# lamortenera/bamsignals

Measured on AMD Instinct MI355X. Metric: Mbases profiled/sec (bamProfile binsize=1), higher is better.
Workload: dtype int32

## Files before the change

### bamsignals_amd/csrc/bsig_types.h

```cpp
#ifndef BSIG_TYPES_H
#define BSIG_TYPES_H
#include <stdint.h>

#define BSIG_MAX_CLASSES 5
#define BSIG_SPAN_CLASSES 4
#define BSIG_CLASS_PACKED 4
#define BSIG_PACK_POS_BITS 15
#define BSIG_PACK_CODES 512
#define BSIG_REF_UNIT_SHIFT 16

struct BsigClassCols {
    const int32_t *pos;
    const int32_t *end;
    const uint32_t *fm;
    const int32_t *tlen;
    const uint32_t *idx;
    int64_t n;
    int32_t maxspan;
    int32_t kshift;
};

struct BsigReadsDev {
    BsigClassCols cls[BSIG_MAX_CLASSES];
    const uint32_t *fmtab;
    int32_t n_codes;
};

struct BsigWorkItem {
    int32_t loc;
    int32_t len;
// ... 18 lines not shown
    uint32_t requiredF;
    uint32_t filteredF;
    int32_t has_tlen_filter;
    int32_t tf0, tf1;
    int32_t use_tlen;
    int32_t shift;
    int32_t midpoint;
    int32_t tspan;
    int32_t ss;
    int32_t binsize;
    uint32_t div_magic;
    int32_t div_shift;
    uint32_t div_m15;
    int32_t div_s15;
    int32_t rel24;
    int32_t ext;
    int32_t tile_cells;
    int32_t accumulate;
    int32_t resolved;
    int32_t cov_reps;
    const uint8_t *ptab;
    int32_t *overflow;
};

#endif
```

### bamsignals_amd/csrc/kernels.h

```cpp
#ifndef BSIG_KERNELS_H
#define BSIG_KERNELS_H
#include <hip/hip_runtime.h>
#include <stdint.h>

#include "../../include/bamsignals_abi.h"
#include "bsig_types.h"

namespace bsig {

struct ScatterPtrs {
    int32_t *pos[BSIG_MAX_CLASSES];
    int32_t *end[BSIG_MAX_CLASSES];
    uint32_t *fm[BSIG_MAX_CLASSES];
    int32_t *tlen[BSIG_MAX_CLASSES];
    uint32_t *gb[BSIG_MAX_CLASSES];
    int32_t kshift[BSIG_MAX_CLASSES];
};

hipError_t launch_pileup(int mode, int ss, int threads, const BsigReadsDev &R, const BsigKParams &P,
                         const BsigWorkItem *items, int64_t n_items, int tile_cells,
                         void *windows ,
                         bool resolve_first ,
                         int32_t *out, hipStream_t st);
hipError_t launch_make_ptab(const BsigReadsDev &R, const BsigKParams &P, uint8_t *out, hipStream_t st);
hipError_t launch_resolve(const BsigReadsDev &R, const BsigKParams &P, int mode, const BsigWorkItem *items,
                          int64_t n_items, void *windows, hipStream_t st);
hipError_t launch_count_heavy(const void *windows, int64_t n_items, int64_t heavy_reads,
                              unsigned long long *count, hipStream_t st);
hipError_t launch_cigar_end(int64_t n, const int32_t *pos, const uint16_t *flag, const int64_t *cigar_off,
                            const uint32_t *cigar, int32_t *end_out, hipStream_t st);
int64_t prep_chunks(int64_t n);
hipError_t launch_pair_sample(int64_t n, const int32_t *pos, const int32_t *end, const uint16_t *flag, const uint8_t *mapq,
                              uint32_t *hist, uint2 *pairs, uint32_t cap, uint32_t *n_pairs, hipStream_t st);
hipError_t launch_codemap_fill(const uint32_t *fmtab, int n_codes, uint16_t *codemap, hipStream_t st);
hipError_t launch_span_hist(int64_t n, int32_t n_ref, const int64_t *ref_off, const uint32_t *ref_units, const int32_t *pos,
                            const int32_t *end, const uint16_t *flag, const uint8_t *mapq, const uint16_t *codemap ,
                            uint32_t *chunk_counts,
                            int32_t *maxspan , hipStream_t st);
// ... 15 lines not shown
```

### bamsignals_amd/csrc/kernels.hip

```cpp
#include <hip/hip_runtime.h>
#include <type_traits>
#include <stdint.h>
#include <stdlib.h>

#include <algorithm>

#include "bsig_types.h"
#include "kernels.h"

#ifdef BSIG_STAMPS
__device__ unsigned long long *g_stamp_buf = nullptr;
__device__ int g_ablate = 0;
#define BSIG_STAMP(k)                                                                       \
    do {                                                                                    \
        if (g_stamp_buf && threadIdx.x == 0) {                                              \
            unsigned long long t_;                                                          \
            asm volatile("s_memrealtime %0\n\ts_waitcnt lgkmcnt(0)" : "=s"(t_)::"memory");    \
            g_stamp_buf[(size_t)blockIdx.x * 8 + (k)] = t_;                                 \
        }                                                                                   \
    } while (0)
#define BSIG_ABLATE(bit) (g_ablate & (bit))
#else
#define BSIG_STAMP(k) do { } while (0)
#define BSIG_ABLATE(bit) 0
// ... 96 lines not shown
            if (TL) {
                const int a = tl < 0 ? -tl : tl;
                if (P.has_tlen_filter) rj |= ((a < P.tf0) | (a > P.tf1)) ? 0xFFFFFFFFu : 0u;
                if (P.midpoint) h = (uint32_t)(a >> 1);
            }
            const uint32_t fwd = d + h + (nm & (sp + cd - 2u * h));
            const uint32_t lc = (REV ? (uint32_t)K - fwd : (uint32_t)K + fwd) | rj;
            const bool ok = (dj + k < nj) & (lc < (uint32_t)nc);
            const uint32_t cell = SS ? (uint32_t)sh + 2u * lc + ((REV ? ~nm : nm) & 1u) : (uint32_t)sh + lc;
            if (ok) atomicAdd(&cnt[cell >> 1], 1u << ((cell << 4) & 31u));
        };
        rd(w.x, b0, t.x, 0u);
        rd(w.y, b1, t.y, 1u);
        rd(w.z, b2, t.z, 2u);
        rd(w.w, b3, t.w, 3u);
    }
};

template <bool SS>
struct SmallOne {
    const BsigKParams &P;
    int32_t *mine;
    int loc, len, c0, nc;
    bool neg_range;
    __device__ __forceinline__ void operator()(int p, int e, bool neg, bool rej, int tl, bool valid) const
    {
        constexpr int S = SS ? 2 : 1;
        if (!valid || rej || tlen_rejected(P, tl)) return;
        const int a = tl < 0 ? -tl : tl;
        const int offset = P.midpoint ? (a >> 1) + P.shift : P.shift;
// ... 206 lines not shown
    }
}
__global__ __launch_bounds__(128) void k_make_ptab(const BsigReadsDev R, const BsigKParams P, uint8_t *__restrict__ out)
{
    const int v = threadIdx.x;
    uint32_t word = 0;
    if (4 * v < R.n_codes) {
        const uint4 f = reinterpret_cast<const uint4 *>(R.fmtab)[v];
        auto b = [&](uint32_t fm) { return (uint32_t)fm_rejected(P, fm) | ((fm >> 3) & 2u); };
        word = b(f.x) | b(f.y) << 8 | b(f.z) << 16 | b(f.w) << 24;
    }
    reinterpret_cast<uint32_t *>(out)[v] = word;
}
static_assert(BSIG_PACK_CODES == 4 * 128, "k_make_ptab: four codes per thread of one 128-thread workgroup");

struct PackedWin {
    int base;
    int n_chunks;
};

__device__ __forceinline__ bool class_window(const BsigClassCols &C, const BsigWorkItem &w,
                                             int64_t tlo, int64_t thi, int ext,
                                             uint32_t &j_lo, uint32_t &j_hi)
{
    int64_t wlo = tlo - ext - C.maxspan + 1;
    int64_t whi = thi + ext;
    const int64_t ref_bp = (int64_t)(w.units_strand & BSIG_ITEM_UNITS_MASK) << BSIG_REF_UNIT_SHIFT;
    if (wlo < 0) wlo = 0;
    if (whi > ref_bp) whi = ref_bp;
    if (wlo >= whi) return false;
// ... 110 lines not shown
        else one.quad(w, t, j - j_lo, nj, base, ptab);
        return;
    }
    const uint32_t b0 = ptab[w.x >> 23], b1 = ptab[w.y >> 23], b2 = ptab[w.z >> 23], b3 = ptab[w.w >> 23];
    const uint32_t dj = j - j_lo;
    auto dec = [&](uint32_t x, uint32_t b, int tl, bool valid) {
        const int pos = base + (int)((x - (uint32_t)base) & kPackPosMask);
        one(pos, pos + (int)((x >> BSIG_PACK_POS_BITS) & 0xFFu), (b & 2u) != 0u, (b & 1u) != 0u, tl, valid);
    };
    dec(w.x, b0, t.x, dj < nj);
    dec(w.y, b1, t.y, dj + 1u < nj);
    dec(w.z, b2, t.z, dj + 2u < nj);
    dec(w.w, b3, t.w, dj + 3u < nj);
}

template <int NT, int kPre = 2, typename Tab, typename F>
__device__ __forceinline__ void for_each_read(const BsigReadsDev &R, const BsigKParams &P,
                                              const uint2 (&win)[BSIG_MAX_CLASSES], int pbase,
                                              const Tab *__restrict__ ptab, int tid, F &&one)
{
    uint4 w0[kPre];
    int4 t0[kPre];
    const BsigClassCols &CP = R.cls[BSIG_CLASS_PACKED];
    const uint32_t jbp = (win[BSIG_CLASS_PACKED].x & ~3u) + 4u * tid;
#pragma unroll
    for (int k = 0; k < kPre; ++k) {
        const uint32_t j = jbp + 4u * NT * k;
        if (j < win[BSIG_CLASS_PACKED].y) {
            w0[k] = *reinterpret_cast<const uint4 *>(CP.fm + j);
            if (P.use_tlen) t0[k] = *reinterpret_cast<const int4 *>(CP.tlen + j);
        }
    }
    const bool small0 = win[0].y - win[0].x <= (uint32_t)NT, small1 = win[1].y - win[1].x <= (uint32_t)NT;
    int pa = 0, ta = 0, pb = 0, tb = 0;
    uint32_t fa = 0, fb = 0;
    const uint32_t jb0 = win[0].x + (uint32_t)tid, jb1 = win[1].x + (uint32_t)tid;
    if (small0 && jb0 < win[0].y) {
        pa = R.cls[0].pos[jb0];
        fa = R.cls[0].fm[jb0];
        if (P.use_tlen) ta = R.cls[0].tlen[jb0];
    }
    if (small1 && jb1 < win[1].y) {
        pb = R.cls[1].pos[jb1];
        fb = R.cls[1].fm[jb1];
        if (P.use_tlen) tb = R.cls[1].tlen[jb1];
    }
    {
        const uint32_t j_lo = win[BSIG_CLASS_PACKED].x, j_hi = win[BSIG_CLASS_PACKED].y, nj = j_hi - j_lo;
        const uint32_t jp0 = j_lo & ~3u;
        auto inner_pass = [&](uint32_t first) { return first >= j_lo && first + 4u * NT <= j_hi; };
#pragma unroll
        for (int k = 0; k < kPre; ++k) {
            const uint32_t j = jbp + 4u * NT * k;
            if (j < j_hi) four_packed(w0[k], t0[k], j, j_lo, nj, pbase, ptab, one, inner_pass(jp0 + 4u * NT * k));
        }
        for (uint32_t j = jbp + 4u * NT * kPre, jf = jp0 + 4u * NT * kPre; j < j_hi; j += 8u * NT, jf += 8u * NT) {
            const uint32_t j2 = j + 4u * NT;
            const uint4 wa = *reinterpret_cast<const uint4 *>(CP.fm + j);
            int4 xa, xb;
            uint4 wb = make_uint4(0, 0, 0, 0);
            if (P.use_tlen) xa = *reinterpret_cast<const int4 *>(CP.tlen + j);
            if (j2 < j_hi) {
// ... 192 lines not shown
    for (int c = 0; c < BSIG_MAX_CLASSES; ++c) { r.win[2 * c] = win[c].x; r.win[2 * c + 1] = win[c].y; }
    r.pbase = pk.base;
    r.pchunks = pk.n_chunks;
    out[t] = r;
}

__device__ __forceinline__ void add_vec(int32_t *__restrict__ gbase, int v, int4 x, int sh, int nv)
{
    const int e0 = 4 * v, lo = sh, hi = sh + nv;
    if (x.x && e0 + 0 >= lo && e0 + 0 < hi) atomicAdd(gbase + e0 + 0, x.x);
    if (x.y && e0 + 1 >= lo && e0 + 1 < hi) atomicAdd(gbase + e0 + 1, x.y);
    if (x.z && e0 + 2 >= lo && e0 + 2 < hi) atomicAdd(gbase + e0 + 2, x.z);
    if (x.w && e0 + 3 >= lo && e0 + 3 < hi) atomicAdd(gbase + e0 + 3, x.w);
}

template <int NT, bool SS, int PRE, int WAVES, bool RES>
__global__ __launch_bounds__(NT) __attribute__((amdgpu_waves_per_eu(WAVES, 8))) void k_profile(const BsigWorkItem *__restrict__ items, uint32_t n_tiles,
                                                int32_t *__restrict__ out,
                                                const uint2 *__restrict__ windows,
                                                const BsigReadsDev R, const BsigKParams P)
{
    extern __shared__ __attribute__((aligned(16))) int32_t lds[];
    constexpr int S = SS ? 2 : 1;
    const int tid = threadIdx.x;
    BSIG_STAMP(0);
    const uint32_t tile = tile_of_block(blockIdx.x, n_tiles);
    const BsigWorkItem w = items[tile];
    uint2 win[BSIG_MAX_CLASSES], clip;
    PackedWin pk;
    load_windows<RES>(R, P, BSIG_MODE_PROFILE, w, items, windows, win, tile, pk, clip);
    int4 *lds4 = reinterpret_cast<int4 *>(lds);
    const int img_vec = (P.tile_cells * S + 8 + 7) / 8;
    for (int v = tid; v < img_vec; v += NT) lds4[v] = make_int4(0, 0, 0, 0);
    uint8_t *ptab = reinterpret_cast<uint8_t *>(lds4 + img_vec);
    build_ptab<NT>(ptab, R, P, tid);
    const int nv = w.nc * S;
    const int sh = (int)(w.out_off & 3);
    const int nvec = (sh + nv + 3) >> 2;
    block_sync<NT>();
    BSIG_STAMP(1);

    const bool neg_range = (w.units_strand & BSIG_ITEM_NEG) != 0u;
    uint32_t *cnt = reinterpret_cast<uint32_t *>(lds);

    const ProfileOne<SS> one{P, cnt, w.loc, w.len, w.c0, w.nc, sh, neg_range};
    if (!BSIG_ABLATE(1)) {
        for_each_read<NT, PRE>(R, P, win, pk.base, ptab, tid, one);
        if (pk.n_chunks > 1) packed_later_chunks<NT>(R, P, BSIG_MODE_PROFILE, w, pk.n_chunks, clip, ptab, tid, one);
    }
    block_sync<NT>();
    BSIG_STAMP(2);

    int32_t *gbase = out + (w.out_off - sh);
    const uint2 *lds2 = reinterpret_cast<const uint2 *>(lds);
    auto widen = [](uint2 d) {
        return make_int4((int)(d.x & 0xFFFFu), (int)(d.x >> 16), (int)(d.y & 0xFFFFu), (int)(d.y >> 16));
    };
    if (P.accumulate) {
        for (int v = tid; v < nvec; v += NT) add_vec(gbase, v, widen(lds2[v]), sh, nv);
    } else if (!BSIG_ABLATE(2)) {
        for (int v = tid; v < nvec; v += NT) store_vec(gbase, v, widen(lds2[v]), sh, nv);
    }
    BSIG_STAMP(3);
#ifdef BSIG_STAMPS
    asm volatile("s_waitcnt vmcnt(0)" ::: "memory");
    BSIG_STAMP(4);
    if (g_stamp_buf && threadIdx.x == 0) {
        unsigned xcc;
        asm volatile("s_getreg_b32 %0, hwreg(HW_REG_XCC_ID)" : "=s"(xcc));
        unsigned hwid;
        asm volatile("s_getreg_b32 %0, hwreg(HW_REG_HW_ID)" : "=s"(hwid));
        g_stamp_buf[(size_t)blockIdx.x * 8 + 5] = ((unsigned long long)xcc << 32) | hwid;
    }
#endif
}

template <bool SS, int PRE, int WAVES, int T>
__global__ __launch_bounds__(kWave) __attribute__((amdgpu_waves_per_eu(WAVES, 8))) void k_profile_multi(
    const BsigWorkItem *__restrict__ items, uint32_t n_tiles, int32_t *__restrict__ out, const uint2 *__restrict__ windows,
    const BsigReadsDev R, const BsigKParams P)
{
    extern __shared__ __attribute__((aligned(16))) int32_t lds[];
    constexpr int S = SS ? 2 : 1;
    constexpr int kStage = 20;
    const int tid = threadIdx.x;
    const uint32_t n_groups = (n_tiles + T - 1) / T;
    const uint32_t first = tile_of_block(blockIdx.x, n_groups) * T;
    const uint32_t n_here = n_tiles - first < (uint32_t)T ? n_tiles - first : (uint32_t)T;
    int4 *lds4 = reinterpret_cast<int4 *>(lds);
    const int img_vec = (P.tile_cells * S + 8 + 7) / 8;
    uint8_t *ptab = reinterpret_cast<uint8_t *>(lds4 + img_vec);
    uint32_t *stage = reinterpret_cast<uint32_t *>(ptab + BSIG_PACK_CODES);
    if ((uint32_t)tid < n_here) {
        const uint4 *ip = reinterpret_cast<const uint4 *>(items + first + tid);
        const uint4 *rp = reinterpret_cast<const uint4 *>(reinterpret_cast<const BsigResolved *>(windows) + first + tid);
        const uint4 a = ip[0], b = ip[1], c = rp[0], d = rp[1], e = rp[2];
        uint4 *sp = reinterpret_cast<uint4 *>(stage + kStage * tid);
        sp[0] = a; sp[1] = b; sp[2] = c; sp[3] = d; sp[4] = e;
    }
    for (int v = tid; v < img_vec; v += kWave) lds4[v] = make_int4(0, 0, 0, 0);
    build_ptab<kWave>(ptab, R, P, tid);
    block_sync<kWave>();
    uint32_t *cnt = reinterpret_cast<uint32_t *>(lds);
    uint2 *lds2 = reinterpret_cast<uint2 *>(lds);
#pragma unroll 1
    for (uint32_t t = 0; t < n_here; ++t) {
        const uint32_t *sg = stage + kStage * t;
        auto sc = [&](int k) { return __builtin_amdgcn_readfirstlane((int)sg[k]); };
        BsigWorkItem w;
        w.loc = sc(0); w.len = sc(1); w.c0 = sc(2); w.nc = sc(3);
        w.out_off = (int64_t)(((uint64_t)(uint32_t)sc(5) << 32) | (uint32_t)sc(4));
        w.ref_unit0 = (uint32_t)sc(6); w.units_strand = (uint32_t)sc(7);
        uint2 win[BSIG_MAX_CLASSES];
#pragma unroll
        for (int c = 0; c < BSIG_MAX_CLASSES; ++c) win[c] = make_uint2((uint32_t)sc(8 + 2 * c), (uint32_t)sc(9 + 2 * c));
        const int pbase = sc(18), pchunks = sc(19);
        const int nv = w.nc * S;
        const int sh = (int)(w.out_off & 3);
        const int nvec = (sh + nv + 3) >> 2;
        const bool neg_range = (w.units_strand & BSIG_ITEM_NEG) != 0u;
        const ProfileOne<SS> one{P, cnt, w.loc, w.len, w.c0, w.nc, sh, neg_range};
        for_each_read<kWave, PRE>(R, P, win, pbase, ptab, tid, one);
        if (pchunks > 1) packed_later_chunks<kWave>(R, P, BSIG_MODE_PROFILE, w, pchunks, make_uint2(0u, 0xFFFFFFFFu), ptab, tid, one);
        block_sync<kWave>();
        int32_t *gbase = out + (w.out_off - sh);
        for (int v = tid; v < nvec; v += kWave) {
            const uint2 d = lds2[v];
            lds2[v] = make_uint2(0u, 0u);
            store_vec(gbase, v, make_int4((int)(d.x & 0xFFFFu), (int)(d.x >> 16), (int)(d.y & 0xFFFFu), (int)(d.y >> 16)), sh, nv);
        }
        block_sync<kWave>();
    }
}

constexpr int kSmallCells = 256;
__host__ __device__ inline int small_replicas(int stride)
{
    return stride <= 32 ? 4 : stride <= 64 ? 2 : 1;
}
__host__ __device__ inline int small_image_dwords(int stride_max)
{
    int most = stride_max * small_replicas(stride_max);
    if (stride_max > 31) most = most > 31 * small_replicas(31) ? most : 31 * small_replicas(31);
    if (stride_max > 63) most = most > 63 * small_replicas(63) ? most : 63 * small_replicas(63);
    return most;
}
template <int NT, bool SS, bool RES>
// ... 718 lines not shown
                streamed += ((j_hi + 3u) & ~3u) - (j_lo & ~3u);
                const uint32_t x = lower_bound_packed(C.fm, j_lo, j_hi, a, wlo);
                const uint32_t y = lower_bound_packed(C.fm, x, j_hi, a, whi);
                v += y - x;
            }
            if (v) atomicAdd(&acc[BSIG_CLASS_PACKED], v);
        }
    }
    atomicAdd(&acc[BSIG_MAX_CLASSES], streamed);
}

}

namespace bsig {

static int g_knobs[6] = {-1, -1, -1, -1, -1, -1};
static int knob(int k)
{
    static const char *const names[6] = {"BAMSIGNALS_PROFILE_PRE", "BAMSIGNALS_COUNT_TILES", "BAMSIGNALS_COUNT_PRE", "BAMSIGNALS_KNOB3",
                                         "BAMSIGNALS_KNOB4", "BAMSIGNALS_PROFILE_TILES"};
    static const int dflt[6] = {2, 0, 0, 0, 0, 0};
    if (g_knobs[k] < 0) {
        const char *e = getenv(names[k]);
        g_knobs[k] = e ? atoi(e) : dflt[k];
    }
    return g_knobs[k];
}

template <int NT>
static hipError_t launch_mode(int mode, int ss, const BsigReadsDev &R, const BsigKParams &P,
                              const BsigWorkItem *items, int64_t n_items, int tile_cells,
                              uint2 *windows, bool resolve_first, int32_t *out, hipStream_t st)
{
    if (n_items <= 0) return hipSuccess;
    const bool count_large = n_items >= 65536;
    const int count_tiles = knob(1) > 0 ? knob(1) : count_large ? 8 : 4, count_pre = knob(2) > 0 ? knob(2) : count_large ? 4 : 2;
// ... 2 lines not shown
        Q.resolved = 0;
        hipLaunchKernelGGL(k_resolve_tiles, dim3((unsigned)((n_items + 255) / 256)), dim3(256), 0, st,
                           R, Q, mode, items, (uint32_t)n_items, reinterpret_cast<BsigResolved *>(windows));
    }
    const dim3 grid((unsigned)n_items), block(NT);
    if (mode == BSIG_MODE_PROFILE && tile_cells * (ss ? 2 : 1) <= kSmallCells && P.binsize > 1) {
        const int stride = (tile_cells * (ss ? 2 : 1)) | 1;
        const size_t lds = (size_t)((small_image_dwords(stride) + 3) & ~3) * sizeof(int32_t) + BSIG_PACK_CODES;
#define BSIG_KS(SS_, RES_) hipLaunchKernelGGL((k_profile_small<NT, SS_, RES_>), grid, block, lds, st, items, (uint32_t)n_items, out, windows, R, P)
        if (ss) { if (P.resolved) BSIG_KS(true, true); else BSIG_KS(true, false); }
        else    { if (P.resolved) BSIG_KS(false, true); else BSIG_KS(false, false); }
#undef BSIG_KS
    } else if (mode == BSIG_MODE_PROFILE) {
        const size_t lds = (size_t)((tile_cells * (ss ? 2 : 1) + 8 + 7) / 8) * 16 + BSIG_PACK_CODES;
        const int pre = knob(0);
#define BSIG_KP(SS_, PRE_, W_)                                                                                                          \
    do {                                                                                                                                \
        if (P.resolved) hipLaunchKernelGGL((k_profile<NT, SS_, PRE_, W_, true>), grid, block, lds, st, items, (uint32_t)n_items, out, windows, R, P); \
        else hipLaunchKernelGGL((k_profile<NT, SS_, PRE_, W_, false>), grid, block, lds, st, items, (uint32_t)n_items, out, windows, R, P); \
    } while (0)
        const bool w8 = NT == kWave && P.resolved && (knob(3) == 8 || (knob(3) == 0 && lds <= 3072));
        const int pt = knob(5) == 0 ? (lds <= 2048 ? 4 : 1) : knob(5);
        if (NT == kWave && P.resolved && !P.accumulate && pt > 1) {
            const int T = pt >= 4 ? 4 : 2;
            const dim3 g2((unsigned)((n_items + T - 1) / T));
            const size_t lds_m = lds + (size_t)T * 20 * sizeof(uint32_t);
#define BSIG_KM(SS_, W_, T_) hipLaunchKernelGGL((k_profile_multi<SS_, 2, W_, T_>), g2, dim3(kWave), lds_m, st, items, (uint32_t)n_items, out, windows, R, P)
            if (ss) { if (w8) { if (T == 4) BSIG_KM(true, 8, 4); else BSIG_KM(true, 8, 2); } else { if (T == 4) BSIG_KM(true, 1, 4); else BSIG_KM(true, 1, 2); } }
            else    { if (w8) { if (T == 4) BSIG_KM(false, 8, 4); else BSIG_KM(false, 8, 2); } else { if (T == 4) BSIG_KM(false, 1, 4); else BSIG_KM(false, 1, 2); } }
#undef BSIG_KM
            return hipGetLastError();
        }
        if (ss) { if (pre <= 2) { if (w8) BSIG_KP(true, 2, 8); else BSIG_KP(true, 2, 1); } else if (pre == 3) BSIG_KP(true, 3, 1); else BSIG_KP(true, 4, 1); }
        else    { if (pre <= 2) { if (w8) BSIG_KP(false, 2, 8); else BSIG_KP(false, 2, 1); } else if (pre == 3) BSIG_KP(false, 3, 1); else BSIG_KP(false, 4, 1); }
#undef BSIG_KP
    } else if (mode == BSIG_MODE_COVERAGE && (P.binsize > 1 || ss)) {
        const int S = ss ? 2 : 1;
        BsigKParams Q = P;
        Q.cov_reps = cov_bins_reps(tile_cells * S);
        const size_t lds = (size_t)cov_bins_vec(tile_cells * S) * Q.cov_reps * 16 + (size_t)((S * NT / 64 + 3) / 4) * 16 + BSIG_PACK_CODES;
#define BSIG_KB(RES_, SS_) hipLaunchKernelGGL((k_coverage_bins<NT, 2, RES_, SS_>), grid, block, lds, st, items, (uint32_t)n_items, out, windows, R, Q)
        if (ss) { if (P.resolved) BSIG_KB(true, true); else BSIG_KB(false, true); }
        else    { if (P.resolved) BSIG_KB(true, false); else BSIG_KB(false, false); }
#undef BSIG_KB
    } else if (mode == BSIG_MODE_COVERAGE) {
        const size_t lds = (size_t)((tile_cells + 8 + 7) / 8) * 16 + (size_t)((NT / 64 + 3) / 4) * 16 + BSIG_PACK_CODES;
        if (P.resolved) hipLaunchKernelGGL((k_coverage<NT, 2, true>), grid, block, lds, st, items, (uint32_t)n_items, out, windows, R, P);
        else hipLaunchKernelGGL((k_coverage<NT, 2, false>), grid, block, lds, st, items, (uint32_t)n_items, out, windows, R, P);
    } else if (NT == kWave && (!windows || P.resolved) && count_tiles > 1) {
// ... 16 lines not shown
{
    switch (threads) {
    case 64:  return launch_mode<64>(mode, ss, R, P, items, n_items, tile_cells, (uint2 *)windows, resolve_first, out, st);
    case 128: return launch_mode<128>(mode, ss, R, P, items, n_items, tile_cells, (uint2 *)windows, resolve_first, out, st);
    case 256: return launch_mode<256>(mode, ss, R, P, items, n_items, tile_cells, (uint2 *)windows, resolve_first, out, st);
    default:  return hipErrorInvalidValue;
    }
}

hipError_t launch_make_ptab(const BsigReadsDev &R, const BsigKParams &P, uint8_t *out, hipStream_t st)
{
    hipLaunchKernelGGL(k_make_ptab, dim3(1), dim3(128), 0, st, R, P, out);
    return hipGetLastError();
}

hipError_t launch_resolve(const BsigReadsDev &R, const BsigKParams &P, int mode, const BsigWorkItem *items,
                          int64_t n_items, void *windows, hipStream_t st)
{
    if (n_items <= 0) return hipSuccess;
    hipLaunchKernelGGL(k_resolve, dim3((unsigned)((n_items * BSIG_MAX_CLASSES + 255) / 256)), dim3(256), 0, st,
                       R, P, mode, items, n_items, (uint2 *)windows);
    return hipGetLastError();
}

hipError_t launch_count_heavy(const void *windows, int64_t n_items, int64_t heavy_reads,
                              unsigned long long *count, hipStream_t st)
{
    if (n_items <= 0) return hipSuccess;
    hipLaunchKernelGGL(k_count_heavy, dim3((unsigned)((n_items + 255) / 256)), dim3(256), 0, st,
                       (const uint2 *)windows, n_items, heavy_reads, count);
// ... 94 lines not shown
}

}

namespace { __global__ void k_warm_pileup() {} }
hipError_t bsig::warm_pileup_module(hipStream_t st)
{
    hipLaunchKernelGGL(k_warm_pileup, dim3(1), dim3(64), 0, st);
    return hipGetLastError();
}

extern "C" int bsig_debug_set_resolve_min(long long n_tiles);
extern "C" int bsig_debug_set_knob(int which, int value)
{
    if (which == 4) return bsig_debug_set_resolve_min(value);
    if (which < 0 || which >= 6 || value < 0) return -1;
    bsig::g_knobs[which] = value;
    return 0;
}

extern "C" int bsig_debug_pileup_attrs(int which, int *vgprs, int *scratch_bytes)
{
    const void *f = nullptr;
    switch (which) {
    case 0: f = reinterpret_cast<const void *>(&k_profile<64, false, 2, 1, true>); break;
    case 1: f = reinterpret_cast<const void *>(&k_profile<64, false, 2, 8, true>); break;
    case 2: f = reinterpret_cast<const void *>(&k_profile<64, false, 2, 1, false>); break;
    case 3: f = reinterpret_cast<const void *>(&k_profile_multi<false, 2, 8, 4>); break;
    case 4: f = reinterpret_cast<const void *>(&k_coverage<64, 2, true>); break;
    case 5: f = reinterpret_cast<const void *>(&k_count_multi<4, 2>); break;
    case 6: f = reinterpret_cast<const void *>(&k_profile<64, true, 2, 1, true>); break;
    default: return 1;
    }
    hipFuncAttributes a;
    if (hipFuncGetAttributes(&a, f) != hipSuccess) return 2;
    if (vgprs) *vgprs = a.numRegs;
    if (scratch_bytes) *scratch_bytes = (int)a.localSizeBytes;
    return 0;
}
#ifdef BSIG_STAMPS
extern "C" int bsig_debug_set_stamp_buffer(void *buf)
{
    return (int)hipMemcpyToSymbol(HIP_SYMBOL(g_stamp_buf), &buf, sizeof(buf));
}
extern "C" int bsig_debug_set_ablate(int bits)
{
// ... 4 lines not shown
```

### bamsignals_amd/csrc/runtime.hip

```cpp
#include <hip/hip_runtime.h>

#include <fcntl.h>
#include <sys/mman.h>
#include <sys/stat.h>
#include <unistd.h>

#include <algorithm>
#include <chrono>
#include <cstdarg>
#include <cstdio>
#include <cstdlib>
#include <cstring>
#include <atomic>
#include <functional>
#include <memory>
#include <mutex>
#include <numeric>
#include <thread>
#include <string>
#include <vector>

#include "../../include/bamsignals_abi.h"
#include "bsig_types.h"
#include "host_util.h"
// ... 350 lines not shown
    HIP_TRY(hipHostMalloc(ptr, (size_t)std::max<int64_t>(bytes, 16), hipHostMallocDefault));
    return BSIG_OK;
}

void bsig_host_free(void *ptr)
{
    if (ptr) (void)hipHostFree(ptr);
}

}

uint64_t bsig::next_layout_gen()
{
    static std::atomic<uint64_t> g{0};
    return ++g;
}

int bsig::layout_from_device(bsig_ctx *ctx, bsig_reads *R, int64_t n, int32_t n_ref, const int32_t *ref_len,
                             const int64_t *ref_off, const int32_t *d_pos, const int32_t *d_end,
                             const uint16_t *d_flag, const uint8_t *d_mapq, const int32_t *d_tlen)
{
    hipStream_t st = ctx->stream;
    HIP_TRY(hipSetDevice(ctx->device));
    R->layout_gen = next_layout_gen();

    R->n_ref = n_ref;
    R->ref_unit0.resize(n_ref);
    R->ref_units.resize(n_ref);
    R->ref_len.assign(ref_len, ref_len + n_ref);
    uint64_t total_units = 0;
// ... 136 lines not shown
        R->info.class_bucket_shift[c] = k;
        R->info.n_classes += 1;
    }
    R->info.n_codes = R->dev.n_codes;

    if (diag) fprintf(stderr, "  [layout] column + index allocations %.1f ms\n", diag_ms());
    HIP_TRY(bsig::launch_scatter(n, n_ref, d_ref_off, d_unit0, d_units, d_pos, d_end, d_flag, d_mapq, d_tlen, d_codemap,
                                 d_base, S, st));
    for (int c = 0; c < BSIG_MAX_CLASSES; ++c)
        if (class_n[c])
            HIP_TRY(bsig::launch_build_idx((int64_t)class_n[c], S.gb[c], n_buckets[c],
                                           const_cast<uint32_t *>(R->dev.cls[c].idx), st));
    HIP_TRY(hipStreamSynchronize(st));
    if (diag) fprintf(stderr, "  [layout] scatter + indexes %.1f ms\n", diag_ms());
    R->info.hbm_bytes = R->pool.footprint();
    return BSIG_OK;
}

extern "C" {

static int upload_impl(bsig_ctx *ctx, const bsig_columns *cols, bsig_reads *R)
{
    const int64_t n = cols->n_reads;
    hipStream_t st = ctx->stream;
    HIP_TRY(hipSetDevice(ctx->device));
    for (int r = 0; r < cols->n_ref; ++r)
        if (cols->ref_len[r] < 0) return fail(BSIG_ERR_ARG, "negative length of reference %d", r);
    if (n == 0 || cols->n_ref == 0)
        return bsig::layout_from_device(ctx, R, n, cols->n_ref, cols->ref_len, cols->ref_off, nullptr, nullptr, nullptr,
                                        nullptr, nullptr);
    DevPool tmp;
// ... 108 lines not shown
        copy(S.tlen, cb, &p); D.tlen = (const int32_t *)p;
        copy(S.idx, (size_t)src->idx_entries[c] * sizeof(uint32_t), &p); D.idx = (const uint32_t *)p;
    }
    {
        void *p;
        copy(src->dev.fmtab, BSIG_PACK_CODES * sizeof(uint32_t), &p);
        R->dev.fmtab = (const uint32_t *)p;
    }
    if (e == hipSuccess) e = hipStreamSynchronize(st);
    if (e != hipSuccess) {
        delete R;
        return fail(e == hipErrorOutOfMemory ? BSIG_ERR_NOMEM : BSIG_ERR_DEVICE, "copying the reads to GPU %d failed: %s", ddev,
                    hipGetErrorString(e));
    }
    R->info.hbm_bytes = R->pool.footprint();
    *out = R;
    return BSIG_OK;
}

}

namespace {

struct DownloadStage {
    std::mutex mu;
    hipEvent_t ev[2] = {nullptr, nullptr};
    static constexpr size_t kHalf = 32u << 20;
    int ensure()
    {
        for (int k = 0; k < 2; ++k)
// ... 484 lines not shown
        hipError_t e = hipMemsetAsync(d_bad, 0, sizeof(int), ctx->stream);
        for (int c = 0; c < BSIG_MAX_CLASSES && e == hipSuccess; ++c) {
            const BsigClassCols &C = R->dev.cls[c];
            if (C.n) e = bsig::launch_check_idx(C.idx, R->idx_entries[c] - 2, (uint32_t)C.n, d_bad, ctx->stream);
        }
        if (e == hipSuccess) e = hipMemcpyAsync(&bad, d_bad, sizeof bad, hipMemcpyDeviceToHost, ctx->stream);
        if (e == hipSuccess) e = hipStreamSynchronize(ctx->stream);
        (void)hipFree(d_bad);
        if (e != hipSuccess) return fail(BSIG_ERR_DEVICE, "checking %s failed: %s", path, hipGetErrorString(e));
        if (bad) return fail(BSIG_ERR_FORMAT, "%s is damaged (bucket index)", path);
        uint64_t sum = 0;
        const int rc = layout_checksum(R.get(), &sum);
        if (rc) return rc;
        if (sum != H.checksum) return fail(BSIG_ERR_FORMAT, "%s is damaged (checksum)", path);
    }
    *out = R.release();
    return BSIG_OK;
}

int bsig_plan_create(bsig_ctx *ctx, const bsig_reads *reads, int64_t n, const int32_t *rid,
                     const int32_t *loc, const int32_t *len, const int32_t *strand,
                     const bsig_params *prm, bsig_plan **out)
{
    if (!ctx || !reads || !prm || !out) return fail(BSIG_ERR_ARG, "NULL argument to bsig_plan_create");
    *out = nullptr;
    if (n < 0 || (n > 0 && (!rid || !loc || !len || !strand))) return fail(BSIG_ERR_ARG, "range arrays missing");
    if (prm->mode == BSIG_MODE_COVERAGE_EX && (prm->binsize < 1 || prm->binsize > bsig::kMaxCoverageBin))
        return fail(BSIG_ERR_ARG, prm->binsize < 1 ? "provide a binsize greater or equal to 1"
                                                   : "coverage bins are at most 65536 bases wide (bamProfile / bamCount count at that scale)");
    const bool cov_ex = prm->mode == BSIG_MODE_COVERAGE_EX;
// ... 51 lines not shown
    K.mapqual = prm->mapqual;
    K.requiredF = (uint32_t)prm->requiredF;
    K.filteredF = (uint32_t)prm->filteredF;
    K.has_tlen_filter = prm->n_tlen_filter == 2;
    K.tf0 = prm->tlen_filter[0]; K.tf1 = prm->tlen_filter[1];
    K.shift = mode == BSIG_MODE_COVERAGE ? 0 : prm->shift;
    K.midpoint = mid; K.tspan = tspan;
    K.use_tlen = K.has_tlen_filter || mid || tspan;
    K.ss = mode == BSIG_MODE_COVERAGE ? cov_ss : (prm->ss != 0);
    K.binsize = mode == BSIG_MODE_PROFILE ? prm->binsize : mode == BSIG_MODE_COVERAGE ? cov_bin : 1;
    K.ext = (int32_t)ext;
    K.tile_cells = P->tile_cells;
    {
        const int64_t h_max = mid ? std::max<int64_t>(0, prm->tlen_filter[1]) / 2 : 0;
        K.rel24 = 2 * std::llabs((long long)K.shift) + h_max + (1 << BSIG_PACK_POS_BITS) + 256 < (1ll << 23);
    }
    bsig::magic_u31(K.binsize, &K.div_magic, &K.div_shift);
    K.div_m15 = 0; K.div_s15 = 0;
    if (K.binsize >= 2 && K.binsize <= 8192) {
        int L = 0;
        while ((1 << L) < K.binsize) ++L;
        K.div_s15 = 15 + L;
        K.div_m15 = (uint32_t)((((uint64_t)1 << K.div_s15) + (uint64_t)K.binsize - 1) / (uint64_t)K.binsize);
    }

    const int32_t lay_binsize = mode == BSIG_MODE_COUNT ? -1 : K.binsize;
    P->off.resize(n + 1);
    bsig_layout(n, len, lay_binsize, K.ss, P->off.data());

    std::vector<int64_t> order;
// ... 252 lines not shown
        hipError_t e = hipMemsetAsync(d_acc, 0, sizeof acc, st);
        if (e == hipSuccess) e = bsig::launch_visits(p->reads->dev, p->kp, p->kernel_mode, p->items, p->n_items, d_acc, st);
        if (e == hipSuccess) e = hipMemcpyAsync(acc, d_acc, sizeof acc, hipMemcpyDeviceToHost, st);
        if (e == hipSuccess) e = hipStreamSynchronize(st);
        (void)hipFree(d_acc);
        if (e != hipSuccess) return fail(BSIG_ERR_DEVICE, "visit count failed: %s", hipGetErrorString(e));
        bsig_plan_stats &t = p->stats;
        t.n_ranges = p->n_ranges;
        t.n_items = p->n_items;
        t.cells = p->off.back();
        t.visits_packed = (int64_t)acc[BSIG_CLASS_PACKED];
        t.visits_short = (int64_t)(acc[0] + acc[1]);
        t.visits = (int64_t)(acc[0] + acc[1] + acc[2] + acc[3] + acc[BSIG_CLASS_PACKED]);
        t.streamed = (int64_t)acc[BSIG_MAX_CLASSES];
        t.heavy_tiles = (int32_t)std::min<int64_t>(p->n_heavy_tiles, INT32_MAX);
        t.bytes_per_visit_packed = p->kp.use_tlen ? 8 : 4;
        t.bytes_per_visit_short = p->kp.use_tlen ? 12 : 8;
        t.bytes_per_visit_long = p->kp.use_tlen ? 16 : 12;
        const int64_t per_item = (int64_t)sizeof(BsigWorkItem);
        t.algorithmic_bytes = t.bytes_per_visit_packed * t.visits_packed + t.bytes_per_visit_short * t.visits_short +
                              t.bytes_per_visit_long * (t.visits - t.visits_short - t.visits_packed) + per_item * t.n_items + 4 * t.cells;
        if (plan_two_launches(p) && windows_kept()) {
            t.algorithmic_bytes += (int64_t)sizeof(BsigResolved) * t.n_items;
        } else {
            t.algorithmic_bytes += 8 * t.n_items * p->reads->info.n_classes;
            if (plan_two_launches(p)) t.algorithmic_bytes += (per_item + 2 * (int64_t)sizeof(BsigResolved)) * t.n_items;
        }
        p->have_stats = true;
    }
    *s = p->stats;
    return BSIG_OK;
// ... 35 lines not shown
```

Baseline: 1.093 million.

## Add precomputed 16-bit packed read column for unfiltered binsize-1 profiles

Builds a per-read 16-bit column at load time that holds the 5' position offset and the strand bit for the packed class. When profile mode uses binsize 1, no tlen filtering, and every flag code passes the filters, new half kernels stream eight reads per 16-byte load. They also skip building the per-tile code table. This halves bytes per packed visit and removes the table lookup and decode work, at the cost of extra HBM, a setup kernel, and a fallback whenever the conditions fail.

```diff
diff --git a/bamsignals_amd/csrc/bsig_types.h b/bamsignals_amd/csrc/bsig_types.h
--- a/bamsignals_amd/csrc/bsig_types.h
+++ b/bamsignals_amd/csrc/bsig_types.h
@@ -14,6 +14,7 @@
     const int32_t *end;
     const uint32_t *fm;
     const int32_t *tlen;
+    const uint16_t *p5h;
     const uint32_t *idx;
     int64_t n;
     int32_t maxspan;
@@ -62,6 +63,7 @@
     uint32_t div_m15;
     int32_t div_s15;
     int32_t rel24;
+    int32_t packed_half;
     int32_t ext;
     int32_t tile_cells;
     int32_t accumulate;
diff --git a/bamsignals_amd/csrc/kernels.h b/bamsignals_amd/csrc/kernels.h
--- a/bamsignals_amd/csrc/kernels.h
+++ b/bamsignals_amd/csrc/kernels.h
@@ -22,6 +22,7 @@
                          void *windows ,
                          bool resolve_first ,
                          int32_t *out, hipStream_t st);
+hipError_t launch_make_p5h(const uint32_t *fm, const uint32_t *fmtab, int64_t n, int64_t cap, uint16_t *out, hipStream_t st);
 hipError_t launch_make_ptab(const BsigReadsDev &R, const BsigKParams &P, uint8_t *out, hipStream_t st);
 hipError_t launch_resolve(const BsigReadsDev &R, const BsigKParams &P, int mode, const BsigWorkItem *items,
                           int64_t n_items, void *windows, hipStream_t st);
diff --git a/bamsignals_amd/csrc/kernels.hip b/bamsignals_amd/csrc/kernels.hip
--- a/bamsignals_amd/csrc/kernels.hip
+++ b/bamsignals_amd/csrc/kernels.hip
@@ -134,6 +134,29 @@
         rd(w.y, b1, t.y, 1u);
         rd(w.z, b2, t.z, 2u);
         rd(w.w, b3, t.w, 3u);
+    }
+    __device__ __forceinline__ void oct(const uint4 &w, uint32_t dj, uint32_t nj, int base) const
+    {
+        if (neg_range) eight<true>(w, dj, nj, base, len - 1 - c0 - (base - loc + P.shift));
+        else eight<false>(w, dj, nj, base, base - loc + P.shift - c0);
+    }
+    template <bool REV>
+    __device__ __forceinline__ void eight(const uint4 &w, uint32_t dj, uint32_t nj, int base, int K) const
+    {
+        const uint32_t cd = (uint32_t)(-2 * P.shift);
+        auto rd = [&](uint32_t h, uint32_t k) {
+            const uint32_t d = (h - (uint32_t)base) & (((uint32_t)1 << BSIG_PACK_POS_BITS) - 1u);
+            const uint32_t nm = (uint32_t)((int32_t)(h << 16) >> 31);
+            const uint32_t fwd = d + (nm & cd);
+            const uint32_t lc = REV ? (uint32_t)K - fwd : (uint32_t)K + fwd;
+            const bool ok = (dj + k < nj) & (lc < (uint32_t)nc);
+            const uint32_t cell = SS ? (uint32_t)sh + 2u * lc + ((REV ? ~nm : nm) & 1u) : (uint32_t)sh + lc;
+            if (ok) atomicAdd(&cnt[cell >> 1], 1u << ((cell << 4) & 31u));
+        };
+        rd(w.x & 0xFFFFu, 0u); rd(w.x >> 16, 1u);
+        rd(w.y & 0xFFFFu, 2u); rd(w.y >> 16, 3u);
+        rd(w.z & 0xFFFFu, 4u); rd(w.z >> 16, 5u);
+        rd(w.w & 0xFFFFu, 6u); rd(w.w >> 16, 7u);
     }
 };
 
@@ -370,6 +393,21 @@
 }
 static_assert(BSIG_PACK_CODES == 4 * 128, "k_make_ptab: four codes per thread of one 128-thread workgroup");
 
+__global__ void k_make_p5h(const uint32_t *__restrict__ fm, const uint32_t *__restrict__ fmtab, int64_t n, int64_t cap,
+                           uint16_t *__restrict__ out)
+{
+    const int64_t i = (int64_t)blockIdx.x * blockDim.x + threadIdx.x;
+    if (i >= cap) return;
+    uint32_t h = 0;
+    if (i < n) {
+        const uint32_t w = fm[i];
+        const uint32_t rev = (fmtab[w >> 23] >> 4) & 1u;
+        const uint32_t p5 = (w & kPackPosMask) + (rev ? (w >> BSIG_PACK_POS_BITS) & 0xFFu : 0u);
+        h = (p5 & kPackPosMask) | rev << 15;
+    }
+    out[i] = (uint16_t)h;
+}
+
 struct PackedWin {
     int base;
     int n_chunks;
@@ -510,21 +548,26 @@
     dec(w.w, b3, t.w, dj + 3u < nj);
 }
 
-template <int NT, int kPre = 2, typename Tab, typename F>
+template <int NT, int kPre = 2, bool HALF = false, typename Tab, typename F>
 __device__ __forceinline__ void for_each_read(const BsigReadsDev &R, const BsigKParams &P,
                                               const uint2 (&win)[BSIG_MAX_CLASSES], int pbase,
                                               const Tab *__restrict__ ptab, int tid, F &&one)
 {
+    constexpr uint32_t kPer = HALF ? 8u : 4u;
     uint4 w0[kPre];
     int4 t0[kPre];
     const BsigClassCols &CP = R.cls[BSIG_CLASS_PACKED];
-    const uint32_t jbp = (win[BSIG_CLASS_PACKED].x & ~3u) + 4u * tid;
+    const uint32_t jbp = (win[BSIG_CLASS_PACKED].x & ~(kPer - 1u)) + kPer * tid;
 #pragma unroll
     for (int k = 0; k < kPre; ++k) {
-        const uint32_t j = jbp + 4u * NT * k;
+        const uint32_t j = jbp + kPer * NT * k;
         if (j < win[BSIG_CLASS_PACKED].y) {
-            w0[k] = *reinterpret_cast<const uint4 *>(CP.fm + j);
-            if (P.use_tlen) t0[k] = *reinterpret_cast<const int4 *>(CP.tlen + j);
+            if constexpr (HALF) {
+                w0[k] = *reinterpret_cast<const uint4 *>(CP.p5h + j);
+            } else {
+                w0[k] = *reinterpret_cast<const uint4 *>(CP.fm + j);
+                if (P.use_tlen) t0[k] = *reinterpret_cast<const int4 *>(CP.tlen + j);
+            }
         }
     }
     const bool small0 = win[0].y - win[0].x <= (uint32_t)NT, small1 = win[1].y - win[1].x <= (uint32_t)NT;
@@ -541,7 +584,23 @@
         fb = R.cls[1].fm[jb1];
         if (P.use_tlen) tb = R.cls[1].tlen[jb1];
     }
-    {
+    if constexpr (HALF) {
+        (void)t0;
+        const uint32_t j_lo = win[BSIG_CLASS_PACKED].x, j_hi = win[BSIG_CLASS_PACKED].y, nj = j_hi - j_lo;
+#pragma unroll
+        for (int k = 0; k < kPre; ++k) {
+            const uint32_t j = jbp + 8u * NT * k;
+            if (j < j_hi) one.oct(w0[k], j - j_lo, nj, pbase);
+        }
+        for (uint32_t j = jbp + 8u * NT * kPre; j < j_hi; j += 16u * NT) {
+            const uint32_t j2 = j + 8u * NT;
+            const uint4 wa = *reinterpret_cast<const uint4 *>(CP.p5h + j);
+            uint4 wb = make_uint4(0, 0, 0, 0);
+            if (j2 < j_hi) wb = *reinterpret_cast<const uint4 *>(CP.p5h + j2);
+            one.oct(wa, j - j_lo, nj, pbase);
+            if (j2 < j_hi) one.oct(wb, j2 - j_lo, nj, pbase);
+        }
+    } else {
         const uint32_t j_lo = win[BSIG_CLASS_PACKED].x, j_hi = win[BSIG_CLASS_PACKED].y, nj = j_hi - j_lo;
         const uint32_t jp0 = j_lo & ~3u;
         auto inner_pass = [&](uint32_t first) { return first >= j_lo && first + 4u * NT <= j_hi; };
@@ -764,11 +823,9 @@
     if (x.w && e0 + 3 >= lo && e0 + 3 < hi) atomicAdd(gbase + e0 + 3, x.w);
 }
 
-template <int NT, bool SS, int PRE, int WAVES, bool RES>
-__global__ __launch_bounds__(NT) __attribute__((amdgpu_waves_per_eu(WAVES, 8))) void k_profile(const BsigWorkItem *__restrict__ items, uint32_t n_tiles,
-                                                int32_t *__restrict__ out,
-                                                const uint2 *__restrict__ windows,
-                                                const BsigReadsDev R, const BsigKParams P)
+template <int NT, bool SS, int PRE, bool RES, bool HALF>
+__device__ __forceinline__ void profile_tile(const BsigWorkItem *__restrict__ items, uint32_t n_tiles, int32_t *__restrict__ out,
+                                             const uint2 *__restrict__ windows, const BsigReadsDev &R, const BsigKParams &P)
 {
     extern __shared__ __attribute__((aligned(16))) int32_t lds[];
     constexpr int S = SS ? 2 : 1;
@@ -783,7 +840,7 @@
     const int img_vec = (P.tile_cells * S + 8 + 7) / 8;
     for (int v = tid; v < img_vec; v += NT) lds4[v] = make_int4(0, 0, 0, 0);
     uint8_t *ptab = reinterpret_cast<uint8_t *>(lds4 + img_vec);
-    build_ptab<NT>(ptab, R, P, tid);
+    if (!HALF) build_ptab<NT>(ptab, R, P, tid);
     const int nv = w.nc * S;
     const int sh = (int)(w.out_off & 3);
     const int nvec = (sh + nv + 3) >> 2;
@@ -795,8 +852,8 @@
 
     const ProfileOne<SS> one{P, cnt, w.loc, w.len, w.c0, w.nc, sh, neg_range};
     if (!BSIG_ABLATE(1)) {
-        for_each_read<NT, PRE>(R, P, win, pk.base, ptab, tid, one);
-        if (pk.n_chunks > 1) packed_later_chunks<NT>(R, P, BSIG_MODE_PROFILE, w, pk.n_chunks, clip, ptab, tid, one);
+        for_each_read<NT, PRE, HALF>(R, P, win, pk.base, ptab, tid, one);
+        if (!HALF && pk.n_chunks > 1) packed_later_chunks<NT>(R, P, BSIG_MODE_PROFILE, w, pk.n_chunks, clip, ptab, tid, one);
     }
     block_sync<NT>();
     BSIG_STAMP(2);
@@ -824,11 +881,26 @@
     }
 #endif
 }
-
-template <bool SS, int PRE, int WAVES, int T>
-__global__ __launch_bounds__(kWave) __attribute__((amdgpu_waves_per_eu(WAVES, 8))) void k_profile_multi(
-    const BsigWorkItem *__restrict__ items, uint32_t n_tiles, int32_t *__restrict__ out, const uint2 *__restrict__ windows,
-    const BsigReadsDev R, const BsigKParams P)
+template <int NT, bool SS, int PRE, int WAVES, bool RES>
+__global__ __launch_bounds__(NT) __attribute__((amdgpu_waves_per_eu(WAVES, 8))) void k_profile(const BsigWorkItem *__restrict__ items, uint32_t n_tiles,
+                                                int32_t *__restrict__ out,
+                                                const uint2 *__restrict__ windows,
+                                                const BsigReadsDev R, const BsigKParams P)
+{
+    profile_tile<NT, SS, PRE, RES, false>(items, n_tiles, out, windows, R, P);
+}
+template <int NT, bool SS, int PRE, int WAVES, bool RES>
+__global__ __launch_bounds__(NT) __attribute__((amdgpu_waves_per_eu(WAVES, 8))) void k_profile_half(const BsigWorkItem *__restrict__ items, uint32_t n_tiles,
+                                                int32_t *__restrict__ out,
+                                                const uint2 *__restrict__ windows,
+                                                const BsigReadsDev R, const BsigKParams P)
+{
+    profile_tile<NT, SS, PRE, RES, true>(items, n_tiles, out, windows, R, P);
+}
+
+template <bool SS, int PRE, int T, bool HALF>
+__device__ __forceinline__ void profile_multi_tiles(const BsigWorkItem *__restrict__ items, uint32_t n_tiles, int32_t *__restrict__ out,
+                                                    const uint2 *__restrict__ windows, const BsigReadsDev &R, const BsigKParams &P)
 {
     extern __shared__ __attribute__((aligned(16))) int32_t lds[];
     constexpr int S = SS ? 2 : 1;
@@ -849,7 +921,7 @@
         sp[0] = a; sp[1] = b; sp[2] = c; sp[3] = d; sp[4] = e;
     }
     for (int v = tid; v < img_vec; v += kWave) lds4[v] = make_int4(0, 0, 0, 0);
-    build_ptab<kWave>(ptab, R, P, tid);
+    if (!HALF) build_ptab<kWave>(ptab, R, P, tid);
     block_sync<kWave>();
     uint32_t *cnt = reinterpret_cast<uint32_t *>(lds);
     uint2 *lds2 = reinterpret_cast<uint2 *>(lds);
@@ -870,8 +942,8 @@
         const int nvec = (sh + nv + 3) >> 2;
         const bool neg_range = (w.units_strand & BSIG_ITEM_NEG) != 0u;
         const ProfileOne<SS> one{P, cnt, w.loc, w.len, w.c0, w.nc, sh, neg_range};
-        for_each_read<kWave, PRE>(R, P, win, pbase, ptab, tid, one);
-        if (pchunks > 1) packed_later_chunks<kWave>(R, P, BSIG_MODE_PROFILE, w, pchunks, make_uint2(0u, 0xFFFFFFFFu), ptab, tid, one);
+        for_each_read<kWave, PRE, HALF>(R, P, win, pbase, ptab, tid, one);
+        if (!HALF && pchunks > 1) packed_later_chunks<kWave>(R, P, BSIG_MODE_PROFILE, w, pchunks, make_uint2(0u, 0xFFFFFFFFu), ptab, tid, one);
         block_sync<kWave>();
         int32_t *gbase = out + (w.out_off - sh);
         for (int v = tid; v < nvec; v += kWave) {
@@ -881,6 +953,20 @@
         }
         block_sync<kWave>();
     }
+}
+template <bool SS, int PRE, int WAVES, int T>
+__global__ __launch_bounds__(kWave) __attribute__((amdgpu_waves_per_eu(WAVES, 8))) void k_profile_multi(
+    const BsigWorkItem *__restrict__ items, uint32_t n_tiles, int32_t *__restrict__ out, const uint2 *__restrict__ windows,
+    const BsigReadsDev R, const BsigKParams P)
+{
+    profile_multi_tiles<SS, PRE, T, false>(items, n_tiles, out, windows, R, P);
+}
+template <bool SS, int PRE, int WAVES, int T>
+__global__ __launch_bounds__(kWave) __attribute__((amdgpu_waves_per_eu(WAVES, 8))) void k_profile_multi_half(
+    const BsigWorkItem *__restrict__ items, uint32_t n_tiles, int32_t *__restrict__ out, const uint2 *__restrict__ windows,
+    const BsigReadsDev R, const BsigKParams P)
+{
+    profile_multi_tiles<SS, PRE, T, true>(items, n_tiles, out, windows, R, P);
 }
 
 constexpr int kSmallCells = 256;
@@ -1629,12 +1715,12 @@
 
 namespace bsig {
 
-static int g_knobs[6] = {-1, -1, -1, -1, -1, -1};
+static int g_knobs[7] = {-1, -1, -1, -1, -1, -1, -1};
 static int knob(int k)
 {
-    static const char *const names[6] = {"BAMSIGNALS_PROFILE_PRE", "BAMSIGNALS_COUNT_TILES", "BAMSIGNALS_COUNT_PRE", "BAMSIGNALS_KNOB3",
-                                         "BAMSIGNALS_KNOB4", "BAMSIGNALS_PROFILE_TILES"};
-    static const int dflt[6] = {2, 0, 0, 0, 0, 0};
+    static const char *const names[7] = {"BAMSIGNALS_PROFILE_PRE", "BAMSIGNALS_COUNT_TILES", "BAMSIGNALS_COUNT_PRE", "BAMSIGNALS_KNOB3",
+                                         "BAMSIGNALS_KNOB4", "BAMSIGNALS_PROFILE_TILES", "BAMSIGNALS_PROFILE_HALF_PRE"};
+    static const int dflt[7] = {2, 0, 0, 0, 0, 0, 2};
     if (g_knobs[k] < 0) {
         const char *e = getenv(names[k]);
         g_knobs[k] = e ? atoi(e) : dflt[k];
@@ -1667,25 +1753,43 @@
     } else if (mode == BSIG_MODE_PROFILE) {
         const size_t lds = (size_t)((tile_cells * (ss ? 2 : 1) + 8 + 7) / 8) * 16 + BSIG_PACK_CODES;
         const int pre = knob(0);
-#define BSIG_KP(SS_, PRE_, W_)                                                                                                          \
+        const bool half = P.packed_half != 0;
+        const int pre_h = knob(6) <= 1 ? 1 : 2;
+#define BSIG_KP(K_, SS_, PRE_, W_)                                                                                                      \
     do {                                                                                                                                \
-        if (P.resolved) hipLaunchKernelGGL((k_profile<NT, SS_, PRE_, W_, true>), grid, block, lds, st, items, (uint32_t)n_items, out, windows, R, P); \
-        else hipLaunchKernelGGL((k_profile<NT, SS_, PRE_, W_, false>), grid, block, lds, st, items, (uint32_t)n_items, out, windows, R, P); \
+        if (P.resolved) hipLaunchKernelGGL((K_<NT, SS_, PRE_, W_, true>), grid, block, lds, st, items, (uint32_t)n_items, out, windows, R, P); \
+        else hipLaunchKernelGGL((K_<NT, SS_, PRE_, W_, false>), grid, block, lds, st, items, (uint32_t)n_items, out, windows, R, P); \
     } while (0)
+#define BSIG_KPW(K_, SS_, PRE_) do { if (w8) BSIG_KP(K_, SS_, PRE_, 8); else BSIG_KP(K_, SS_, PRE_, 1); } while (0)
         const bool w8 = NT == kWave && P.resolved && (knob(3) == 8 || (knob(3) == 0 && lds <= 3072));
         const int pt = knob(5) == 0 ? (lds <= 2048 ? 4 : 1) : knob(5);
         if (NT == kWave && P.resolved && !P.accumulate && pt > 1) {
             const int T = pt >= 4 ? 4 : 2;
             const dim3 g2((unsigned)((n_items + T - 1) / T));
             const size_t lds_m = lds + (size_t)T * 20 * sizeof(uint32_t);
-#define BSIG_KM(SS_, W_, T_) hipLaunchKernelGGL((k_profile_multi<SS_, 2, W_, T_>), g2, dim3(kWave), lds_m, st, items, (uint32_t)n_items, out, windows, R, P)
-            if (ss) { if (w8) { if (T == 4) BSIG_KM(true, 8, 4); else BSIG_KM(true, 8, 2); } else { if (T == 4) BSIG_KM(true, 1, 4); else BSIG_KM(true, 1, 2); } }
-            else    { if (w8) { if (T == 4) BSIG_KM(false, 8, 4); else BSIG_KM(false, 8, 2); } else { if (T == 4) BSIG_KM(false, 1, 4); else BSIG_KM(false, 1, 2); } }
+#define BSIG_KM(K_, SS_, PRE_, W_, T_) hipLaunchKernelGGL((K_<SS_, PRE_, W_, T_>), g2, dim3(kWave), lds_m, st, items, (uint32_t)n_items, out, windows, R, P)
+#define BSIG_KMT(K_, SS_, PRE_, W_) do { if (T == 4) BSIG_KM(K_, SS_, PRE_, W_, 4); else BSIG_KM(K_, SS_, PRE_, W_, 2); } while (0)
+#define BSIG_KMW(K_, SS_, PRE_) do { if (w8) BSIG_KMT(K_, SS_, PRE_, 8); else BSIG_KMT(K_, SS_, PRE_, 1); } while (0)
+            if (half) {
+                if (ss) { if (pre_h == 1) BSIG_KMW(k_profile_multi_half, true, 1); else BSIG_KMW(k_profile_multi_half, true, 2); }
+                else    { if (pre_h == 1) BSIG_KMW(k_profile_multi_half, false, 1); else BSIG_KMW(k_profile_multi_half, false, 2); }
+            } else {
+                if (ss) BSIG_KMW(k_profile_multi, true, 2);
+                else    BSIG_KMW(k_profile_multi, false, 2);
+            }
+#undef BSIG_KMW
+#undef BSIG_KMT
 #undef BSIG_KM
             return hipGetLastError();
         }
-        if (ss) { if (pre <= 2) { if (w8) BSIG_KP(true, 2, 8); else BSIG_KP(true, 2, 1); } else if (pre == 3) BSIG_KP(true, 3, 1); else BSIG_KP(true, 4, 1); }
-        else    { if (pre <= 2) { if (w8) BSIG_KP(false, 2, 8); else BSIG_KP(false, 2, 1); } else if (pre == 3) BSIG_KP(false, 3, 1); else BSIG_KP(false, 4, 1); }
+        if (half) {
+            if (ss) { if (pre_h == 1) BSIG_KPW(k_profile_half, true, 1); else BSIG_KPW(k_profile_half, true, 2); }
+            else    { if (pre_h == 1) BSIG_KPW(k_profile_half, false, 1); else BSIG_KPW(k_profile_half, false, 2); }
+            return hipGetLastError();
+        }
+        if (ss) { if (pre <= 2) BSIG_KPW(k_profile, true, 2); else if (pre == 3) BSIG_KP(k_profile, true, 3, 1); else BSIG_KP(k_profile, true, 4, 1); }
+        else    { if (pre <= 2) BSIG_KPW(k_profile, false, 2); else if (pre == 3) BSIG_KP(k_profile, false, 3, 1); else BSIG_KP(k_profile, false, 4, 1); }
+#undef BSIG_KPW
 #undef BSIG_KP
     } else if (mode == BSIG_MODE_COVERAGE && (P.binsize > 1 || ss)) {
         const int S = ss ? 2 : 1;
@@ -1732,6 +1836,13 @@
     return hipGetLastError();
 }
 
+hipError_t launch_make_p5h(const uint32_t *fm, const uint32_t *fmtab, int64_t n, int64_t cap, uint16_t *out, hipStream_t st)
+{
+    if (cap <= 0) return hipSuccess;
+    hipLaunchKernelGGL(k_make_p5h, dim3((unsigned)((cap + 255) / 256)), dim3(256), 0, st, fm, fmtab, n, cap, out);
+    return hipGetLastError();
+}
+
 hipError_t launch_resolve(const BsigReadsDev &R, const BsigKParams &P, int mode, const BsigWorkItem *items,
                           int64_t n_items, void *windows, hipStream_t st)
 {
@@ -1856,7 +1967,7 @@
 extern "C" int bsig_debug_set_knob(int which, int value)
 {
     if (which == 4) return bsig_debug_set_resolve_min(value);
-    if (which < 0 || which >= 6 || value < 0) return -1;
+    if (which < 0 || which >= 7 || value < 0) return -1;
     bsig::g_knobs[which] = value;
     return 0;
 }
@@ -1872,6 +1983,10 @@
     case 4: f = reinterpret_cast<const void *>(&k_coverage<64, 2, true>); break;
     case 5: f = reinterpret_cast<const void *>(&k_count_multi<4, 2>); break;
     case 6: f = reinterpret_cast<const void *>(&k_profile<64, true, 2, 1, true>); break;
+    case 7: f = reinterpret_cast<const void *>(&k_profile_half<64, false, 2, 1, true>); break;
+    case 8: f = reinterpret_cast<const void *>(&k_profile_half<64, false, 1, 1, true>); break;
+    case 9: f = reinterpret_cast<const void *>(&k_profile_multi_half<false, 2, 8, 4>); break;
+    case 10: f = reinterpret_cast<const void *>(&k_profile_half<64, true, 2, 1, true>); break;
     default: return 1;
     }
     hipFuncAttributes a;
diff --git a/bamsignals_amd/csrc/runtime.hip b/bamsignals_amd/csrc/runtime.hip
--- a/bamsignals_amd/csrc/runtime.hip
+++ b/bamsignals_amd/csrc/runtime.hip
@@ -388,6 +388,22 @@
 {
     static std::atomic<uint64_t> g{0};
     return ++g;
+}
+
+static int make_packed_half(bsig_reads *R, hipStream_t st)
+{
+    BsigClassCols &C = R->dev.cls[BSIG_CLASS_PACKED];
+    C.p5h = nullptr;
+    const char *e = getenv("BAMSIGNALS_PACKED_HALF");
+    if (C.n == 0 || !R->dev.fmtab || (e && !strcmp(e, "0"))) return BSIG_OK;
+    const int64_t cap = (C.n + 7) / 8 * 8 + 8;
+    uint16_t *p = nullptr;
+    HIP_TRY(R->pool.alloc(&p, (size_t)cap));
+    HIP_TRY(bsig::launch_make_p5h(C.fm, R->dev.fmtab, C.n, cap, p, st));
+    HIP_TRY(hipStreamSynchronize(st));
+    C.p5h = p;
+    R->info.hbm_bytes = R->pool.footprint();
+    return BSIG_OK;
 }
 
 int bsig::layout_from_device(bsig_ctx *ctx, bsig_reads *R, int64_t n, int32_t n_ref, const int32_t *ref_len,
@@ -554,7 +570,7 @@
     HIP_TRY(hipStreamSynchronize(st));
     if (diag) fprintf(stderr, "  [layout] scatter + indexes %.1f ms\n", diag_ms());
     R->info.hbm_bytes = R->pool.footprint();
-    return BSIG_OK;
+    return make_packed_half(R, st);
 }
 
 extern "C" {
@@ -693,6 +709,10 @@
                     hipGetErrorString(e));
     }
     R->info.hbm_bytes = R->pool.footprint();
+    if (const int rc = make_packed_half(R, st)) {
+        delete R;
+        return rc;
+    }
     *out = R;
     return BSIG_OK;
 }
@@ -1207,6 +1227,7 @@
         if (rc) return rc;
         if (sum != H.checksum) return fail(BSIG_ERR_FORMAT, "%s is damaged (checksum)", path);
     }
+    if (const int rc = make_packed_half(R.get(), ctx->stream)) return rc;
     *out = R.release();
     return BSIG_OK;
 }
@@ -1288,6 +1309,18 @@
     {
         const int64_t h_max = mid ? std::max<int64_t>(0, prm->tlen_filter[1]) / 2 : 0;
         K.rel24 = 2 * std::llabs((long long)K.shift) + h_max + (1 << BSIG_PACK_POS_BITS) + 256 < (1ll << 23);
+    }
+    {
+        const BsigClassCols &C = reads->dev.cls[BSIG_CLASS_PACKED];
+        bool half = mode == BSIG_MODE_PROFILE && K.binsize == 1 && !K.use_tlen && C.p5h != nullptr;
+        for (int c = 0; half && c < reads->dev.n_codes; ++c) {
+            const uint32_t fm = reads->fmtab[(size_t)c];
+            const uint32_t nf = ~(fm & 0xFFFFu);
+            const bool rej = (int)((fm >> 16) & 0xFFu) < K.mapqual || (K.requiredF & nf) != 0u || (K.filteredF & nf) == 0u;
+            half = !rej;
+        }
+        half = half && (int64_t)K.tile_cells + 2 * ext + C.maxspan + 2 * ((int64_t)1 << C.kshift) <= (1 << BSIG_PACK_POS_BITS) - 256;
+        K.packed_half = half ? 1 : 0;
     }
     bsig::magic_u31(K.binsize, &K.div_magic, &K.div_shift);
     K.div_m15 = 0; K.div_s15 = 0;
@@ -1570,7 +1603,7 @@
         t.visits = (int64_t)(acc[0] + acc[1] + acc[2] + acc[3] + acc[BSIG_CLASS_PACKED]);
         t.streamed = (int64_t)acc[BSIG_MAX_CLASSES];
         t.heavy_tiles = (int32_t)std::min<int64_t>(p->n_heavy_tiles, INT32_MAX);
-        t.bytes_per_visit_packed = p->kp.use_tlen ? 8 : 4;
+        t.bytes_per_visit_packed = p->kp.packed_half ? 2 : p->kp.use_tlen ? 8 : 4;
         t.bytes_per_visit_short = p->kp.use_tlen ? 12 : 8;
         t.bytes_per_visit_long = p->kp.use_tlen ? 16 : 12;
         const int64_t per_item = (int64_t)sizeof(BsigWorkItem);
```

New measurement: 1.151 million, median of 6. 1.05x the previous value.
